# ebartrum/lightning_gan_zoo

Measured on AMD Instinct MI355X. Metric: images/sec (G+D step) at 64x64 bs=128/GPU, higher is better.
Workload: dtype f32; 1 GPU; dc_gan synthetic 64x64 bs=128/GPU, one optimizer cycle of 2 batches (Lightning alternation + toggle), reference optimizer, fp32; key=dc_gan_bs128, global_batch=128, parallelism=dp1, images_counted=2*bs*n_gpus per step (every batch of the cycle)

## Files before the change

### lightning_gan_zoo_amd/csrc/gz_conv.hip

```cpp
#include <cstdio>
#include <type_traits>

#include "gz_conv_choice.h"
#include "gz_conv_direct.h"
#include "gz_igemm.h"
#include "gz_reduce.h"
#include "../../include/gz_ops.h"

namespace gz {


static TileId pick_tile2(long long M, long long N, int ny, int kdim) {
    const bool off = knobs().no_igemm2;
    if (!off && N > 32 && N <= 64 && kdim >= 256) {
        const long long t = ((M + 511) / 512) * ny;
        if (t >= 2 * cus()) return T512x64;
        if (!knobs().no_tile64 && knobs().igemm2_tile == 0 && N == 64 && ((M + 255) / 256) * ny >= cus()) return T256x64;
        return T64x64;
    }
    if (off || N < 128 || kdim < 256) return T64x64;
    const long long t128 = ((M + 255) / 256) * ((N + 127) / 128) * ny;
    const long long t256 = ((M + 255) / 256) * ((N + 255) / 256) * ny;
    const int force = knobs().igemm2_tile;
    const int cu = cus();
// ... 1013 lines not shown
    size_t fewc = 0;
    if (KH == 4 && KW == 4 && wgrad_k4s2p1_fewc_ok(s)) fewc = (size_t)wgrad_k4s2p1_fewc_blocks(s) * (count + K) * 4;
    int chunks = (N * OH * OW + BK - 1) / BK;
    long long tiles = (long long)((K + 127) / 128) * ((C * KH * KW + 127) / 128);
    int splits = wgrad_splits(tiles, chunks);
    {
        const int s2 = (KH == 4 && KW == 4) ? wgrad2_splits<G4421>(s)
                       : (KH == 5 && KW == 5 && OH * 2 == H) ? wgrad2_splits<G5522>(s)
                       : (KH == 3 && KW == 3 && OH == H) ? wgrad2_splits<G3311>(s) : 0;
        if (s2 > splits) splits = s2;
    }
    const size_t generic = splits > 1 ? (size_t)splits * count * 4 : 0;
    return generic > fewc ? generic : fewc;
}

int gz_conv2d_wgrad_fuses_bias(int N, int C, int H, int W, int K, int OH, int OW, int KH, int KW, int S, int P) {
    ConvShape s{N, C, H, W, K, OH, OW};
    if (!shape_ok(s, KH, KW, S, P)) return 0;
#define CALL(G) choose_wgrad<G>(s, kIdeal)
    const Choice c = [&]() -> Choice { GZ_GEOM_DISPATCH_OR(CALL, choice_of(KUnsupported, LGeneric, T64x64)) }();
#undef CALL
    return c.kind == KDirect && c.loader != LFewc;
}

int gz_conv2d_wgrad(const float* x, const float* y, float* dw, float* dbias, float* workspace, size_t ws_bytes, int N,
                    int C, int H, int W, int K, int OH, int OW, int KH, int KW, int S, int P, hipStream_t stream) {
    gz::clear_stale_error();
    ConvShape s{N, C, H, W, K, OH, OW};
    if (!shape_ok(s, KH, KW, S, P)) return GZ_ERR_BAD_SHAPE;
    if (too_large((long long)N * C * H * W) || too_large((long long)N * K * OH * OW)) return GZ_ERR_TOO_LARGE;
    const Facts f = facts_of((const void*)((uintptr_t)x | (uintptr_t)y), dw, workspace, ws_bytes, false, false);
#define CALL(G) launch_wgrad<G>(choose_wgrad<G>(s, f), x, y, dw, dbias, workspace, ws_bytes, s, stream)
    GZ_GEOM_DISPATCH(CALL)
#undef CALL
}

int gz_conv2d_wgrad_partial(const float* x, const float* y, float* dw, float* workspace, size_t ws_bytes, int N, int C,
                            int H, int W, int K, int OH, int OW, int KH, int KW, int S, int P, int* nz_out,
                            long long* stride_out, hipStream_t stream) {
    gz::clear_stale_error();
    if (!nz_out || !stride_out) return GZ_ERR_BAD_SHAPE;
    ConvShape s{N, C, H, W, K, OH, OW};
    if (!shape_ok(s, KH, KW, S, P)) return GZ_ERR_BAD_SHAPE;
    if (too_large((long long)N * C * H * W) || too_large((long long)N * K * OH * OW)) return GZ_ERR_TOO_LARGE;
    *nz_out = 1;
    *stride_out = (long long)K * C * KH * KW;
    const Facts f = facts_of((const void*)((uintptr_t)x | (uintptr_t)y), dw, workspace, ws_bytes, false, false);
    WgDefer d{1, *stride_out};
    tl_wg_defer = &d;
#define CALL(G) launch_wgrad<G>(choose_wgrad<G>(s, f), x, y, dw, nullptr, workspace, ws_bytes, s, stream)
    const int rc = [&]() -> int { GZ_GEOM_DISPATCH(CALL) }();
#undef CALL
    tl_wg_defer = nullptr;
    *nz_out = d.nz;
    *stride_out = d.stride;
    return rc;
}

static bool dgrad_act_direct(const ConvShape& s, int KH, int KW, int S, int P, int act) {
    return KH == 4 && KW == 4 && S == 2 && P == 1 && (act == ACT_RELU || act == ACT_LRELU) && !knobs().no_act_fuse &&
           dgrad_direct<G4421>(s) && smallc_four_pos(s);
}

int gz_conv2d_dgrad_act_fuses(int N, int C, int H, int W, int K, int OH, int OW, int KH, int KW, int S, int P, int act) {
    ConvShape s{N, C, H, W, K, OH, OW};
    return shape_ok(s, KH, KW, S, P) && dgrad_act_direct(s, KH, KW, S, P, act) ? 1 : 0;
}

int gz_conv2d_dgrad_act(const float* gy, const float* fwd_out, int act, float slope, const float* wpack, float* x, int N,
                        int C, int H, int W, int K, int OH, int OW, int KH, int KW, int S, int P, hipStream_t stream) {
    gz::clear_stale_error();
    ConvShape s{N, C, H, W, K, OH, OW};
    if (!gy || !fwd_out || !wpack || !x || !shape_ok(s, KH, KW, S, P)) return GZ_ERR_BAD_SHAPE;
    if (too_large((long long)N * C * H * W) || too_large((long long)N * K * OH * OW)) return GZ_ERR_TOO_LARGE;
    if (!dgrad_act_direct(s, KH, KW, S, P, act) || (((uintptr_t)gy | (uintptr_t)x | (uintptr_t)fwd_out | (uintptr_t)wpack) & 15))
        return GZ_ERR_UNSUPPORTED;
    const float neg = act == ACT_RELU ? 0.f : slope;
    const int ks = smallc_split((long long)N * OH * OW / 4, K);
    return run_dgrad_smallc(gy, wpack, nullptr, x, s, ACT_NONE, 0.f, stream, ks, fwd_out, neg);
}

int gz_set_cu_budget(int cu_count) {
    if (cu_count <= 0) cu_count = 256;
    if (cu_count < 64) cu_count = 64;
    if (cu_count > 256) cu_count = 256;
    gz::cu_budget_ref().store(cu_count, std::memory_order_relaxed);
    return cu_count;
}

int gz_get_cu_budget(void) { return gz::cus(); }

static int stats_wm(TileId t) { return t == T128x32 ? 4 : 2; }
static int stats_tm_rows(TileId t, long long M) {
    if (t == T256x256 || t == T256x128) return (int)((M + 255) / 256) * 2;
    if (t == T512x64) return (int)((M + 511) / 512) * 4;
    if (t == T256x64) return (int)((M + 255) / 256) * 2;
    const int bm = t == T64x64 ? 64 : 128;
    return (int)((M + bm - 1) / bm) * stats_wm(t);
}

int gz_conv2d_fwd_stats_rows(int N, int C, int H, int W, int K, int OH, int OW, int KH, int KW, int S, int P) {
    ConvShape s{N, C, H, W, K, OH, OW};
    if (!shape_ok(s, KH, KW, S, P)) return 0;
    const Facts f{true, true, true, kIdeal.ws_bytes, false, true, true};
#define CALL(G) choose_fwd<G>(s, f)
    const Choice sp = [&]() -> Choice { GZ_GEOM_DISPATCH_OR(CALL, (Choice{KIgemm, LGeneric, T64x64, 2})) }();
#undef CALL
    if (sp.splits > 1) return (int)(((long long)N * OH * OW + 31) / 32);
    return stats_tm_rows(sp.tile, (long long)N * OH * OW);
}

int gz_conv2d_fwd_stats_ws(const float* x, const float* wpack, float* y, float* stats, float* workspace, size_t ws_bytes,
                           int N, int C, int H, int W, int K, int OH, int OW, int KH, int KW, int S, int P,
                           hipStream_t stream) {
    gz::clear_stale_error();
    ConvShape s{N, C, H, W, K, OH, OW};
    if (!shape_ok(s, KH, KW, S, P) || !stats) return GZ_ERR_BAD_SHAPE;
    if (gz_conv2d_fwd_stats_rows(N, C, H, W, K, OH, OW, KH, KW, S, P) <= 0) return GZ_ERR_UNSUPPORTED;
    if ((((uintptr_t)x | (uintptr_t)y) & 15) != 0) return GZ_ERR_BAD_SHAPE;
    if (too_large((long long)N * C * H * W) || too_large((long long)N * K * OH * OW)) return GZ_ERR_TOO_LARGE;
    const Facts f = facts_of(x, y, workspace, ws_bytes, false, true);
#define CALL(G) launch_fwd<G>(choose_fwd<G>(s, f), x, wpack, nullptr, y, s, 0, 0.f, workspace, stats, stream)
    GZ_GEOM_DISPATCH(CALL)
#undef CALL
}

int gz_conv2d_fwd_stats(const float* x, const float* wpack, float* y, float* stats, int N, int C, int H, int W, int K,
                        int OH, int OW, int KH, int KW, int S, int P, hipStream_t stream) {
    return gz_conv2d_fwd_stats_ws(x, wpack, y, stats, nullptr, 0, N, C, H, W, K, OH, OW, KH, KW, S, P, stream);
}

int gz_conv2d_dgrad_stats_rows(int N, int C, int H, int W, int K, int OH, int OW, int KH, int KW, int S, int P) {
    ConvShape s{N, C, H, W, K, OH, OW};
    if (!shape_ok(s, KH, KW, S, P) || H % S || W % S) return 0;
    const Facts f{true, true, true, kIdeal.ws_bytes, false, true, true};
#define CALL(G) (dgrad_direct<G>(s) ? Choice{KIgemm, LGeneric, T64x64, 2} : choose_dgrad<G>(s, f))
    const Choice sp = [&]() -> Choice { GZ_GEOM_DISPATCH_OR(CALL, (Choice{KIgemm, LGeneric, T64x64, 2})) }();
#undef CALL
    if (is_tile2(sp.tile) && !(KH == 4 && KW == 4 && S == 2 && P == 1)) return 0;
    if (sp.splits > 1) {
        if (!(KH == 4 && KW == 4 && S == 2 && P == 1)) return 0;
        return S * S * (int)(((long long)N * (H / S) * (W / S) + 31) / 32);
    }
    return S * S * stats_tm_rows(sp.tile, (long long)N * (H / S) * (W / S));
}

int gz_conv2d_dgrad_stats_ws(const float* y, const float* wpack, float* x, float* stats, float* workspace,
                             size_t ws_bytes, int N, int C, int H, int W, int K, int OH, int OW, int KH, int KW, int S,
                             int P, hipStream_t stream) {
    gz::clear_stale_error();
    ConvShape s{N, C, H, W, K, OH, OW};
    if (!shape_ok(s, KH, KW, S, P) || !stats) return GZ_ERR_BAD_SHAPE;
    if (gz_conv2d_dgrad_stats_rows(N, C, H, W, K, OH, OW, KH, KW, S, P) <= 0) return GZ_ERR_UNSUPPORTED;
    if ((((uintptr_t)x | (uintptr_t)y) & 15) != 0) return GZ_ERR_BAD_SHAPE;
    if (too_large((long long)N * C * H * W) || too_large((long long)N * K * OH * OW)) return GZ_ERR_TOO_LARGE;
    const Facts f = facts_of(y, x, workspace, ws_bytes, false, true);
#define CALL(G) launch_dgrad<G>(choose_dgrad<G>(s, f), y, wpack, nullptr, x, s, 0, 0.f, workspace, stats, stream)
    GZ_GEOM_DISPATCH(CALL)
#undef CALL
}

int gz_conv2d_dgrad_stats(const float* y, const float* wpack, float* x, float* stats, int N, int C, int H, int W, int K,
                          int OH, int OW, int KH, int KW, int S, int P, hipStream_t stream) {
    return gz_conv2d_dgrad_stats_ws(y, wpack, x, stats, nullptr, 0, N, C, H, W, K, OH, OW, KH, KW, S, P, stream);
}

static bool any_shape_ok(const ConvShape& s, const AnyGeom& g) {
// ... 160 lines not shown
```

### lightning_gan_zoo_amd/csrc/gz_igemm2.h

```cpp
#pragma once
#include "gz_igemm_core.h"

namespace gz {

constexpr int STAGES2 = 3;
#ifndef GZ2_DEPTH_TN1_KG2
#define GZ2_DEPTH_TN1_KG2 6
#endif
#ifndef GZ2_DEPTH_TN1_KG1
#define GZ2_DEPTH_TN1_KG1 4
#endif
#ifndef GZ2_DEPTH_TN2_KG2
#define GZ2_DEPTH_TN2_KG2 3
#endif
#ifndef GZ2_DEPTH_TN2_KG1
#define GZ2_DEPTH_TN2_KG1 3
#endif
#ifndef GZ2_BARRIER_TN1_KG2
#define GZ2_BARRIER_TN1_KG2 2
#endif
#ifndef GZ2_BARRIER_TN1_KG1
#define GZ2_BARRIER_TN1_KG1 2
#endif
constexpr uint32_t SOFF_OOB = 0x80000000u;

template <int WM_, int WN_, int TN_, int OCC_, int TM_ = 4>
struct TileCfg2 {
    static constexpr int WM = WM_, WN = WN_, TM = TM_, TN = TN_, OCC = OCC_;
    static constexpr int BM = WM * TM * 32, BN = WN * TN * 32;
    static_assert(WM * WN == 4, "4 wavefronts per workgroup, one per SIMD");
};

template <int BN>
struct MContigB2 {
    static_assert(BN == 64 || BN == 128 || BN == 256, "piece mapping");
    using Params = typename MContigLoader<BN>::Params;
    static constexpr int LD = BN, ROWS = BK;
    static constexpr int PIECES = BK * BN / 256 / 4;
    static constexpr int RPP = 256 / BN;
    __amdgpu_buffer_rsrc_t rsrc;
    uint32_t voff, ldb;
    int wave;
    __device__ __forceinline__ void init(const Params& p, int tile, int y, int tid) {
        rsrc = make_rsrc(p.base + (long long)y * p.batch_stride, (uint32_t)p.K * p.ld * 4u);
        const int lane = tid & 63;
        wave = __builtin_amdgcn_readfirstlane(tid >> 6);
        const int f = lane * 4, r = f / BN, col = f % BN;
        const int n = tile * BN + col;
        ldb = (uint32_t)p.ld * 4u;
        voff = n < p.MN ? (uint32_t)(r * p.ld + n) * 4u : OOB;
    }
    __device__ __forceinline__ void issue_piece(int kc, float* stage, int p, bool live) {
        const int piece = wave * PIECES + p;
        bload_lds16(rsrc, stage + piece * 256, voff, live ? (uint32_t)(kc * BK + piece * RPP) * ldb : SOFF_OOB);
    }
};

template <int BM>
struct ConvDgA2 {
    static_assert(BM == 256 || BM == 512, "whole 256-pixel pieces per LDS row");
    using Params = typename ConvDgALoader<BM, 4, 4, 2, 1>::Params;
    static constexpr int PPR = BM / 256;
    static constexpr int LD = BM + 4, ROWS = BK / 2, PIECES = 2 * PPR;
    static constexpr int ZERO_COL = BM;
    static constexpr bool ROWSHARE = true;
    __amdgpu_buffer_rsrc_t rsrc;
    uint32_t voff[2 * PPR];
    int wave, K, OHW, shift_half1;
    __device__ __forceinline__ void init(const Params& p, int tile, int phase, int tid) {
        const ConvShape& s = p.s;
        rsrc = make_rsrc(p.y, (uint32_t)s.N * s.K * s.OH * s.OW * 4u);
        const int lane = tid & 63;
        wave = __builtin_amdgcn_readfirstlane(tid >> 6);
        K = s.K; OHW = s.OH * s.OW;
        const int py = phase / 2, px = phase % 2;
        shift_half1 = (px + 1) / 2 - 1;
#pragma unroll
        for (int hb = 0; hb < PPR; ++hb) {
            const uint32_t m = (uint32_t)tile * BM + hb * 256 + lane * 4;
            const bool m_ok = m < (uint32_t)s.N * p.AH * p.AW;
            const uint32_t n = fdiv(m, p.div_ahw);
            const uint32_t pix = m - n * (uint32_t)(p.AH * p.AW);
            const uint32_t a = fdiv(pix, p.div_aw);
            const uint32_t b = pix - a * (uint32_t)p.AW;
#pragma unroll
            for (int ty = 0; ty < 2; ++ty) {
                const int oy = (int)a + (py + 1) / 2 - ty;
                const bool ok = m_ok && (unsigned)oy < (unsigned)s.OH;
                voff[ty * PPR + hb] = ok ? (n * (uint32_t)(s.K * OHW) + (uint32_t)(oy * s.OW) + b) * 4u : OOB;
            }
        }
    }
    __device__ __forceinline__ int frag_shift(int half) const { return half ? shift_half1 : shift_half1 + 1; }
    __device__ __forceinline__ void issue_piece(int kc, float* stage, int p, bool live) {
        const int kol = kc * (BK / 4) + wave;
        bload_lds16(rsrc, stage + (wave * 2 + p / PPR) * LD + (p % PPR) * 256, voff[p],
                    (live && kol < K) ? (uint32_t)kol * (uint32_t)OHW * 4u : SOFF_OOB);
    }
};

template <int BM, int OWC>
struct ConvFwdA2 {
    static_assert(BM == 256 && BM % OWC == 0 && OWC >= 2, "piece mapping");
    using Params = typename ConvFwdALoader<BM, 4, 4, 2, 1>::Params;
    static constexpr int LD = BM, ROWS = BK / 2, PIECES = 2;
    static constexpr int OW_C = OWC;
    static constexpr int EXTRA = (6 * OWC + 4 + 3) & ~3;
    static constexpr bool FWDROWS = true;
    __amdgpu_buffer_rsrc_t rsrc;
    uint32_t voff[2];
    int wave, HW, C;
    __device__ __forceinline__ void init(const Params& p, int tile, int y, int tid) {
        const ConvShape& s = p.s;
        rsrc = make_rsrc(p.x, (uint32_t)(s.N * s.C * s.H * s.W) * 4u);
        const int lane = tid & 63;
        wave = __builtin_amdgcn_readfirstlane(tid >> 6);
        HW = s.H * s.W; C = s.C;
#pragma unroll
        for (int q = 0; q < 2; ++q) {
            const int f = ((wave * 2 + q) * 64 + lane) * 4;
            const int seg = f / (8 * OWC), rem = f - seg * 8 * OWC;
            const int ky = rem / (2 * OWC), col = rem - ky * 2 * OWC;
            const uint32_t m = (uint32_t)tile * BM + seg * OWC;
            const bool m_ok = m < (uint32_t)s.N * s.OH * s.OW;
            const uint32_t n = fdiv(m, p.div_ohw);
            const uint32_t oy = fdiv(m - n * (uint32_t)(s.OH * s.OW), p.div_ow);
            const int iy = (int)oy * 2 - 1 + ky;
            const bool ok = m_ok && (unsigned)iy < (unsigned)s.H;
            voff[q] = ok ? (n * (uint32_t)(s.C * HW) + (uint32_t)(iy * s.W + col)) * 4u : OOB;
        }
    }
    static constexpr int ZERO = ROWS * LD;
    __device__ __forceinline__ void frag(int m_local, int half, int& even, int& odd) const {
        const int seg = m_local / OWC, ox = m_local - seg * OWC;
        const int base = seg * 8 * OWC + 2 * ox - 1 + half;
        even = (half == 0 && ox == 0) ? ZERO : base;
        odd = (half == 1 && ox == OWC - 1) ? ZERO : base + 2;
    }
    __device__ __forceinline__ void issue_piece(int kc, float* stage, int p, bool live) {
        bload_lds16(rsrc, stage + (wave * 2 + p) * 256, voff[p], (live && kc < C) ? (uint32_t)kc * (uint32_t)HW * 4u : SOFF_OOB);
    }
};

template <class Geo_>
struct TapGatherA2 {
    using Geo = Geo_;
    using Params = typename Geo::Params;
    static constexpr int BM = Geo::BM, LD = BM, ROWS = BK;
    static constexpr int G = BM / 64;
    static constexpr int PIECES = BK * G / 4;
    Geo geo;
    __amdgpu_buffer_rsrc_t rsrc;
    uint32_t vbase[G], veff[G];
    typename Geo::Pix pix[G];
    int wave, blocks, last_tap, last_kc, cb;
    uint32_t tap_soff;
    __device__ __forceinline__ void init(const Params& p, int tile, int y, int tid) {
        rsrc = geo.init(p, y);
        const int lane = tid & 63;
        wave = __builtin_amdgcn_readfirstlane(tid >> 6);
        blocks = round_bk(geo.chans) / BK;
        last_tap = -1; last_kc = -1; cb = 0; tap_soff = 0;
#pragma unroll
        for (int g = 0; g < G; ++g) {
            vbase[g] = geo.locate(p, (uint32_t)tile * BM + g * 64 + lane, pix[g]);
            veff[g] = OOB;
        }
    }
    __device__ __forceinline__ void issue_piece(int kc, float* stage, int p, bool live) {
        if (p == 0) {
            int tap = last_tap;
            if (kc == last_kc + 1 && last_kc >= 0) {
                cb += BK;
                if (cb >= blocks * BK) { cb = 0; ++tap; }
            } else {
                tap = kc / blocks;
                cb = (kc - tap * blocks) * BK;
            }
            last_kc = kc;
            if (tap != last_tap) {
                last_tap = tap;
                const auto tp = geo.tap(tap);
                tap_soff = geo.tap_bytes(tp);
#pragma unroll
                for (int g = 0; g < G; ++g) veff[g] = geo.inside(pix[g], tp) ? vbase[g] : OOB;
            }
        }
        const int row = wave * 4 + p / G, g = p % G;
        const int c = cb + row;
        bload_lds4(rsrc, stage + row * LD + g * 64, veff[g],
                   (live && c < geo.chans) ? (uint32_t)c * (uint32_t)geo.plane * 4u + tap_soff : SOFF_OOB);
    }
};

template <int BM, int KH, int KW, int S, int P>
using ConvTapA2 = TapGatherA2<TapGeoFwd<BM, KH, KW, S, P>>;
template <int BM>
using ConvTapAnyA2 = TapGatherA2<TapGeoFwdAny<BM>>;
template <int BM, int KH, int KW, int S, int P>
using ConvDgTapA2 = TapGatherA2<TapGeoDg<BM, KH, KW, S, P>>;
template <int BM, int KS, int S, int P>
using Conv3DTapA2 = TapGatherA2<TapGeoFwd3D<BM, KS, S, P>>;
template <int BM, int KS, int S, int P>
using Conv3DDgTapA2 = TapGatherA2<TapGeoDg3D<BM, KS, S, P>>;

template <int BM>
struct ConvDg5A2 {
    static_assert(BM == 256, "one 256-pixel piece per LDS row");
    using Params = typename ConvDgALoaderTap<BM, 5, 5, 2, 2>::Params;
    static constexpr int LD = BM + 4, ROWS = 8, PIECES = 2;
    static constexpr int ZERO_COL = BM;
    static constexpr bool ROWSHARE = true, DUALMODE = true;
    static constexpr int MODES = 2, KSTEPS = 12;
    static constexpr bool step_plain(int m, int S) { return S >= 8; }
    static constexpr unsigned step_mask(int m, int S) {
        return m == 0 ? (S < 8 ? 15u : 5u) : (S < 8 ? 3u : 1u);
    }
    static constexpr int step_arow(int m, int S) { return S < 8 ? S : 2 * (S - 8); }
    static constexpr int step_brow(int m, int S) { return S < 8 ? 2 * S : 16 + 2 * (S - 8); }
    __amdgpu_buffer_rsrc_t rsrc;
    uint32_t voff0, voff1, voff2;
    int wave, K, OHW;
    int bound[1];
// ... 165 lines not shown
                 : "v"(a), "v"(b[0]), "v"(b[1]), "v"(b[2]), "v"(b[3]));
}
__device__ __forceinline__ void mfma_row_mn(f32x16 (&c)[2], float a, const float (&b)[2]) {
    asm volatile(GZ2_NOP
                 "v_mfma_f32_32x32x2_f32 %0, %2, %3, %0\n\t"
                 "v_mfma_f32_32x32x2_f32 %1, %2, %4, %1"
                 : "+a"(c[0]), "+a"(c[1])
                 : "v"(a), "v"(b[0]), "v"(b[1]));
}
__device__ __forceinline__ void lgkm_done(float (&a)[4], float (&b)[4]) {
    asm volatile("s_waitcnt lgkmcnt(0)" : "+v"(a[0]), "+v"(a[1]), "+v"(a[2]), "+v"(a[3]), "+v"(b[0]), "+v"(b[1]), "+v"(b[2]), "+v"(b[3]));
}
__device__ __forceinline__ void lgkm_done(float (&a)[4], float (&b)[2]) {
    asm volatile("s_waitcnt lgkmcnt(0)" : "+v"(a[0]), "+v"(a[1]), "+v"(a[2]), "+v"(a[3]), "+v"(b[0]), "+v"(b[1]));
}
__device__ __forceinline__ void lgkm_done(float (&a)[2], float (&b)[4]) {
    asm volatile("s_waitcnt lgkmcnt(0)" : "+v"(a[0]), "+v"(a[1]), "+v"(b[0]), "+v"(b[1]), "+v"(b[2]), "+v"(b[3]));
}
__device__ __forceinline__ void lgkm_done(float (&a)[4], float (&b)[1]) {
    asm volatile("s_waitcnt lgkmcnt(0)" : "+v"(a[0]), "+v"(a[1]), "+v"(a[2]), "+v"(a[3]), "+v"(b[0]));
}

template <class AL, class = void>
struct a_extra_of { static constexpr int value = 0; };
template <class AL>
struct a_extra_of<AL, std::void_t<decltype(AL::EXTRA)>> { static constexpr int value = AL::EXTRA; };
template <class AL>
constexpr int igemm2_a_extra() { return a_extra_of<AL>::value; }
template <class AL, class = void>
struct fwd_ow_of { static constexpr int value = 1; };
template <class AL>
struct fwd_ow_of<AL, std::void_t<decltype(AL::OW_C)>> { static constexpr int value = AL::OW_C; };
template <class AL>
constexpr int fwd_ow() { return fwd_ow_of<AL>::value; }

template <class AL>
constexpr int mode_count_of() {
    if constexpr (is_dualmode<AL>::value) return AL::MODES;
    else return 1;
}
template <class AL>
constexpr bool mode_plain_of(int m, int S) {
    if constexpr (is_dualmode<AL>::value) return AL::step_plain(m, S);
    else return false;
}
template <class AL>
constexpr unsigned mode_mask_of(int m, int S) {
    if constexpr (is_dualmode<AL>::value) return AL::step_mask(m, S);
    else return 0xFu;
}
template <class AL>
constexpr int ksteps_of() {
    if constexpr (is_dualmode<AL>::value) return AL::KSTEPS;
    else return BK / 2;
}
template <class AL>
constexpr int step_arow_of(int m, int S) {
    if constexpr (is_dualmode<AL>::value) return AL::step_arow(m, S);
    else return S;
}
template <class AL>
constexpr int step_brow_of(int m, int S) {
    if constexpr (is_dualmode<AL>::value) return AL::step_brow(m, S);
    else return 2 * S;
}

constexpr size_t LDS_PER_CU = 160 * 1024;
template <class AL, class BL>
constexpr int igemm2_stage_floats() { return AL::ROWS * AL::LD + igemm2_a_extra<AL>() + BL::ROWS * BL::LD; }
template <class Cfg, class AL, class BL, int KG>
constexpr size_t igemm2_lds_bytes_at(int depth) {
    if (KG == 1) return (size_t)(depth * igemm2_stage_floats<AL, BL>() + 32) * 4;
    const size_t rings = (size_t)(2 * ((depth * igemm2_stage_floats<AL, BL>() + 63) / 64 * 64) + 32) * 4;
    const size_t park = (size_t)Cfg::TM * Cfg::TN * 16 * NT * 4;
    return rings > park ? rings : park;
}
template <class Cfg, class AL, class BL, int KG>
constexpr bool igemm2_tunable() {
    return Cfg::BM == 256 && (is_rowshare<AL>::value || is_fwdrows<AL>::value) && !is_dualmode<AL>::value &&
           fwd_ow<AL>() < 64;
}
template <class Cfg, class AL, class BL, int KG>
constexpr int igemm2_interval() {
    if (igemm2_tunable<Cfg, AL, BL, KG>() && Cfg::TN == 1) return KG == 2 ? GZ2_BARRIER_TN1_KG2 : GZ2_BARRIER_TN1_KG1;
    return 1;
}
template <class Cfg, class AL, class BL, int KG>
constexpr int igemm2_depth() {
    if (igemm2_tunable<Cfg, AL, BL, KG>()) {
        if (Cfg::TN == 1) return KG == 2 ? GZ2_DEPTH_TN1_KG2 : GZ2_DEPTH_TN1_KG1;
        if (Cfg::TN == 2) return KG == 2 ? GZ2_DEPTH_TN2_KG2 : GZ2_DEPTH_TN2_KG1;
    }
    return STAGES2;
}
template <class Cfg, class AL, class BL, int KG>
constexpr int igemm2_ring_floats() {
    return ((igemm2_depth<Cfg, AL, BL, KG>() * igemm2_stage_floats<AL, BL>() + 63) / 64) * 64;
}
template <class Cfg, class AL, class BL>
constexpr size_t igemm2_lds_bytes() { return igemm2_lds_bytes_at<Cfg, AL, BL, 1>(igemm2_depth<Cfg, AL, BL, 1>()); }
template <class Cfg, class AL, class BL>
constexpr size_t igemm2_lds_bytes_kg2() { return igemm2_lds_bytes_at<Cfg, AL, BL, 2>(igemm2_depth<Cfg, AL, BL, 2>()); }

template <class Cfg, class AL, class BL, class Epi, int KG = 1>
__global__ __launch_bounds__(NT * KG, KG == 1 ? Cfg::OCC : 2) void igemm2_kernel(typename AL::Params pa, typename BL::Params pb,
                                                                              typename Epi::Params pe, GridMap gm) {
    constexpr int LDA = AL::LD, LDB = BL::LD;
    constexpr int TM = Cfg::TM, TN = Cfg::TN;
    static_assert((TM == 4 || (TM == 2 && is_dualmode<AL>::value)) && (TN == 1 || TN == 2 || TN == 4),
                  "fragment registers of the hand-ordered k-step");
    static_assert(KG == 1 || (KG == 2 && TN <= 2), "two wave groups: the parked accumulators must fit the LDS");
    constexpr bool RS = is_rowshare<AL>::value;
    constexpr bool FR = is_fwdrows<AL>::value;
    constexpr bool DM = is_dualmode<AL>::value;
    static_assert(!DM || (RS && KG == 1 && (TN == 2 || TN == 4)), "multi-mode: row-shared loader, phases in the accumulator blocks");
    constexpr int A_EXTRA = igemm2_a_extra<AL>();
    constexpr int A_ELEMS = AL::ROWS * LDA + A_EXTRA, B_ELEMS = BL::ROWS * LDB;
    constexpr int STAGE = A_ELEMS + B_ELEMS;
    constexpr int PAD = 16;
    constexpr int DEPTH = igemm2_depth<Cfg, AL, BL, KG>();
    constexpr int BI = igemm2_interval<Cfg, AL, BL, KG>();
    constexpr int GROUPS = DEPTH / BI;
    static_assert(DEPTH % BI == 0 && (BI == 1 ? GROUPS >= 3 : GROUPS >= 2) && (BI == 1 || (BI == 2 && !DM)),
                  "group t+GROUPS-1 lands in the stages group t-1 was read from");
    static_assert(DEPTH == STAGES2 || (KG == 2 ? igemm2_lds_bytes_kg2<Cfg, AL, BL>()
                                               : Cfg::OCC * igemm2_lds_bytes<Cfg, AL, BL>()) <= LDS_PER_CU,
                  "workgroups per CU x LDS per workgroup");
    extern __shared__ __attribute__((aligned(16))) float smem2[];
    const int kg = KG == 1 ? 0 : __builtin_amdgcn_readfirstlane((int)threadIdx.x >> 8);
    float* const ring = smem2 + PAD + kg * igemm2_ring_floats<Cfg, AL, BL, KG>();
    GZ2_STAMP(st0);
#ifdef GZ2_STAMPS
    const unsigned long long sr0 = __builtin_amdgcn_s_memrealtime();
    unsigned long long st1 = st0, st2 = st0;
#endif

    const int tid = KG == 1 ? (int)threadIdx.x : ((int)threadIdx.x & (NT - 1));
    const int nwg = gridDim.x;
    int bid = blockIdx.x;
    if (gm.stagger > 0 && bid < 512 && blockIdx.z == 0) {
        const unsigned hw = __builtin_amdgcn_s_getreg(((4 - 1) << 11) | (16 << 6) | 4);
        if (hw & 1u) {
            const unsigned long long t_end = __builtin_amdgcn_s_memtime() + (unsigned long long)gm.stagger;
            while (__builtin_amdgcn_s_memtime() < t_end) __builtin_amdgcn_s_sleep(64);
        }
    }
    int y;
    if (gm.var_chunks) {
        const int tiles = gm.tiles_m * gm.tiles_n;
        y = gm.phase_order[bid / tiles];
        bid %= tiles;
    } else {
        if (!gm.no_swizzle) {
            const int q = nwg >> 3, rr = nwg & 7, x = bid & 7, i = bid >> 3;
            bid = (x < rr ? x * (q + 1) : rr * (q + 1) + (x - rr) * q) + i;
        }
        y = bid % gm.ny;
        bid /= gm.ny;
    }
    const int tile_n = bid % gm.tiles_n;
    const int tile_m = bid / gm.tiles_n;
    const int z = blockIdx.z;
    const int kcA = z * gm.chunks_per_split;
    const int kcB = min(gm.var_chunks ? gm.phase_chunks[y] : gm.chunks, kcA + gm.chunks_per_split);
    if (gm.slab && gm.var_chunks && kcA >= kcB) return;
    int kc0 = kcA, kc1 = kcB, kend = kcB;
    if constexpr (KG == 2) {
        const int h = (kcB - kcA + 1) >> 1;
        kc0 = kcA + kg * h;
        kend = kc0 + h;
        kc1 = min(kcB, kend);
    }

    AL al;
    BL bl;
    al.init(pa, tile_m, y, tid);
    bl.init(pb, tile_n, y, tid);

    f32x16 acc[TM][TN];
#pragma unroll
    for (int i = 0; i < TM; ++i)
#pragma unroll
        for (int j = 0; j < TN; ++j)
#pragma unroll
            for (int r = 0; r < 16; ++r) acc[i][j][r] = 0.f;

    const int lane = tid & 63, wave = __builtin_amdgcn_readfirstlane(tid >> 6);
    const int wm = wave / Cfg::WN, wn = wave % Cfg::WN;
    const int half = lane >> 5, l32 = lane & 31;
    const uint32_t lds0 = (uint32_t)(uintptr_t)(__attribute__((address_space(3))) float*)ring;
    uint32_t a_addr[TM];
#pragma unroll
    for (int i = 0; i < TM; ++i)
        a_addr[i] = lds0 + (uint32_t)(B_ELEMS + half * (RS ? 0 : LDA) + wm * TM * 32 + i * 32 + l32) * 4u;
    if constexpr (RS) {
        const int sh = al.frag_shift(half);
#pragma unroll
        for (int i = 0; i < TM; ++i) {
            const int b = (tile_m * Cfg::BM + wm * TM * 32 + i * 32 + l32) % pa.AW;
            const bool zero = (sh < 0 && b == 0) || (sh > 0 && b == pa.AW - 1);
            a_addr[i] = zero ? lds0 + (uint32_t)(B_ELEMS + AL::ZERO_COL) * 4u : a_addr[i] + (uint32_t)(sh * 4);
        }
        static_assert(DEPTH * AL::ROWS * 4 <= NT, "one pad float per thread");
        if (tid < DEPTH * AL::ROWS * 4) {
            const int st = tid / (AL::ROWS * 4), q = tid % (AL::ROWS * 4);
            ring[st * STAGE + B_ELEMS + (q >> 2) * LDA + AL::ZERO_COL + (q & 3)] = 0.f;
        }
    }
    uint32_t a_addrB[TM];
    if constexpr (DM) {
#pragma unroll
        for (int i = 0; i < TM; ++i) {
            const int b = (tile_m * Cfg::BM + wm * TM * 32 + i * 32 + l32) % pa.AW;
            a_addrB[i] = lds0 + (uint32_t)(B_ELEMS + half * LDA + (b == 0 ? AL::ZERO_COL : wm * TM * 32 + i * 32 + l32 - 1)) * 4u;
        }
    }
    uint32_t a_odd[TM];
    if constexpr (FR) {
#pragma unroll
        for (int i = 0; i < TM; ++i) {
            int e, o;
            al.frag(wm * TM * 32 + i * 32 + l32, half, e, o);
            a_addr[i] = lds0 + (uint32_t)(B_ELEMS + e) * 4u;
            a_odd[i] = lds0 + (uint32_t)(B_ELEMS + o) * 4u;
        }
        for (int q = tid; q < DEPTH * A_EXTRA; q += NT)
            ring[(q / A_EXTRA) * STAGE + B_ELEMS + AL::ZERO + q % A_EXTRA] = 0.f;
    }
    const uint32_t b_addr = lds0 + (uint32_t)(half * LDB + wn * TN * 32 + l32) * 4u;

    constexpr int NPA = AL::PIECES, NPB = BL::PIECES, NP = NPA + NPB, STEPS = ksteps_of<AL>();
    static_assert((STEPS == 8 || STEPS == 12) && (BI == 1 || STEPS == 8), "k-steps per chunk, per group 8, 12 or 16");
    constexpr int PPS = (NP + STEPS - 1) / STEPS;
    static_assert(PPS <= 4 && (DEPTH - BI) * NP < 64,
                  "pieces are spread over the k-step's four MFMA rows; vmcnt is 6 bits and DEPTH-BI chunks are in flight");
    constexpr int NWAIT = (DEPTH - 2 * BI) * NP;
    constexpr int GSTEPS = BI * STEPS;
    auto issue_piece = [&](int kc, int st, int p, bool live) {
#ifdef GZ2_EXP_NODMA
        if (kc >= kc0 + DEPTH - BI) return;
#endif
#ifdef GZ2_EXP_SAMECHUNK
        if (kc >= kc0 + DEPTH - BI) kc = kc0;
#endif
        float* sb = ring + st * STAGE;
        if (p < NPA) al.issue_piece(kc, sb + B_ELEMS, p, live);
        else bl.issue_piece(kc, sb, p - NPA, live);
    };
    auto fetch_m = [&](auto Sc, auto Mc, uint32_t so, float (&af)[TM], float (&bf)[TN]) {
        constexpr int S = decltype(Sc)::value, MD = decltype(Mc)::value;
        constexpr bool PL = mode_plain_of<AL>(MD, S);
        constexpr unsigned MK = mode_mask_of<AL>(MD, S);
        constexpr int AO = LDA * step_arow_of<AL>(MD, S) * 4, BO = step_brow_of<AL>(MD, S) * LDB * 4;
#pragma unroll
        for (int i = 0; i < TM; ++i) af[i] = lds_rd<AO>((PL ? a_addrB[i] : a_addr[i]) + so);
        if constexpr ((MK & 1u) != 0) bf[0] = lds_rd<BO>(b_addr + so);
        if constexpr (TN >= 2 && (MK & 2u) != 0) bf[1] = lds_rd<BO + 128>(b_addr + so);
        if constexpr (TN == 4 && (MK & 4u) != 0) bf[2] = lds_rd<BO + 256>(b_addr + so);
        if constexpr (TN == 4 && (MK & 8u) != 0) bf[3] = lds_rd<BO + 384>(b_addr + so);
    };
    auto fetch_first = [&](int kc, uint32_t so, float (&af)[TM], float (&bf)[TN]) {
        if constexpr (DM) {
            if (al.mode_of(kc) == 0) fetch_m(std::integral_constant<int, 0>{}, std::integral_constant<int, 0>{}, so, af, bf);
            else fetch_m(std::integral_constant<int, 0>{}, std::integral_constant<int, 1>{}, so, af, bf);
        }
    };
    auto fetch = [&](auto Sc, uint32_t so, float (&af)[TM], float (&bf)[TN]) {
        constexpr int S = decltype(Sc)::value % STEPS, JO = decltype(Sc)::value / STEPS * STAGE * 4;
        constexpr int AO = (RS ? LDA : 2 * LDA) * S * 4 + JO, BO = 2 * S * LDB * 4 + JO;
        static_assert(AO + 2 * LDA * 4 < 65536 && BO + 512 < 65536, "ds_read immediate offsets");
#ifdef GZ2_EXP_NOFETCH
        if (so != 0xFFFFFFFFu) return;
#endif
        if constexpr (FR) {
            constexpr int FO = (S >> 1) * 2 * fwd_ow<AL>() * 4 + JO;
            af[0] = lds_rd<FO>(((S & 1) ? a_odd[0] : a_addr[0]) + so);
            af[1] = lds_rd<FO>(((S & 1) ? a_odd[1] : a_addr[1]) + so);
            af[2] = lds_rd<FO>(((S & 1) ? a_odd[2] : a_addr[2]) + so);
            af[3] = lds_rd<FO>(((S & 1) ? a_odd[3] : a_addr[3]) + so);
        } else {
            af[0] = lds_rd<AO>(a_addr[0] + so);
            af[1] = lds_rd<AO>(a_addr[1] + so);
            af[2] = lds_rd<AO>(a_addr[2] + so);
            af[3] = lds_rd<AO>(a_addr[3] + so);
        }
        {
        bf[0] = lds_rd<BO>(b_addr + so);
        if constexpr (TN >= 2) bf[1] = lds_rd<BO + 128>(b_addr + so);
        if constexpr (TN == 4) {
            bf[2] = lds_rd<BO + 256>(b_addr + so);
            bf[3] = lds_rd<BO + 384>(b_addr + so);
        }
        }
    };
    auto mask = [&](float (&)[TM]) {};

    if (kcA < kcB) {
#pragma unroll
        for (int d = 0; d < DEPTH - BI; ++d)
#pragma unroll
            for (int p = 0; p < NP; ++p) issue_piece(kc0 + d, d, p, kc0 + d < kc1);
#ifdef GZ2_EXP_NO_LGKM_PROLOGUE
        asm volatile("s_waitcnt vmcnt(%0)" ::"n"(NWAIT) : "memory");
#else
        asm volatile("s_waitcnt vmcnt(%0) lgkmcnt(0)" ::"n"(NWAIT) : "memory");
#endif
        __builtin_amdgcn_s_barrier();
#ifdef GZ2_STAMPS
        st1 = __builtin_amdgcn_s_memtime();
#endif
        float af[2][TM], bf[2][TN];
#ifdef GZ2_STEP_STAMPS
        unsigned long long step_cyc[STEPS] = {}, step_t = __builtin_amdgcn_s_memtime();
        unsigned long long wait_cyc[2] = {0, 0};
#endif
        if constexpr (DM) {
#pragma unroll
            for (int q = 0; q < 2; ++q)
#pragma unroll
                for (int j = 0; j < TN; ++j) bf[q][j] = 0.f;
            fetch_first(kc0, 0u, af[0], bf[0]);
        } else {
            fetch(std::integral_constant<int, 0>{}, 0u, af[0], bf[0]);
        }
        lgkm_done(af[0], bf[0]);
        mask(af[0]);
        int stage = 0;
        auto run_chunks = [&](int k_from, int k_to, auto Mc) {
        for (int kc = k_from; kc < k_to; kc += BI) {
            int s1 = stage + 1; if (s1 >= GROUPS) s1 -= GROUPS;
            int s2 = stage - 1; if (s2 < 0) s2 += GROUPS;
            const uint32_t so = (uint32_t)(stage * BI * STAGE * 4), sno = (uint32_t)(s1 * BI * STAGE * 4);
            const bool more = kc + DEPTH - BI < kc1, more1 = kc + DEPTH - BI + 1 < kc1;
            auto kstep = [&](auto Sc) {
                constexpr int S = decltype(Sc)::value;
                constexpr int MD = decltype(Mc)::value;
                constexpr int c = S & 1, n = c ^ 1;
                auto mfma_row = [&](f32x16 (&cc)[TN], float a, const float (&b)[TN]) {
                    if constexpr (DM) {
                        constexpr unsigned MK = mode_mask_of<AL>(MD, S);
                        if constexpr (MK == (TN == 4 ? 15u : 3u)) gz::mfma_row(cc, a, b);
                        else {
                            if constexpr ((MK & 1u) != 0) gz::mfma_one(cc[0], a, b[0]);
                            if constexpr (TN >= 2 && (MK & 2u) != 0) gz::mfma_one(cc[1], a, b[1]);
                            if constexpr (TN == 4 && (MK & 4u) != 0) gz::mfma_one(cc[2], a, b[2]);
                            if constexpr (TN == 4 && (MK & 8u) != 0) gz::mfma_one(cc[3], a, b[3]);
                        }
                    } else gz::mfma_row(cc, a, b);
                };
                auto fetch_same = [&](auto S2c, uint32_t o, float (&fa)[TM], float (&fb)[TN]) {
                    if constexpr (DM) fetch_m(S2c, Mc, o, fa, fb);
                    else fetch(S2c, o, fa, fb);
                };
                auto pieces = [&](auto Rowc) {
                    constexpr int row = decltype(Rowc)::value;
                    constexpr int r = PPS == 1 ? (row == 1 ? 0 : -1) : row;
                    constexpr int q = S * PPS + r;
                    if constexpr (r >= 0 && r < PPS && q < BI * NP)
// ... 717 lines not shown
```

### lightning_gan_zoo_amd/csrc/gz_knobs.h

```cpp
#pragma once
#include <stdlib.h>
#include <string.h>
#include <atomic>

namespace gz {

#define GZ_KNOB_LIST(X)                                                                                               \
                                                                                          \
    X(bool, no_igemm2, "GZ_NO_IGEMM2", false)                        \
    X(bool, no_igemm2_tap, "GZ_NO_IGEMM2_TAP", false)                      \
    X(bool, no_plane_a, "GZ_NO_PLANE_A", false)                \
    X(bool, no_wg3r, "GZ_NO_WG3R", false)                               \
    X(int, wg3r_wgs, "GZ_WG3R_WGS", 2)                              \
    X(int, wg3r_min_chunks, "GZ_WG3R_MIN_CHUNKS", 24)                         \
    X(bool, no_fewk_wg, "GZ_NO_FEWK_WG", false)               \
    X(bool, no_fewk_conv, "GZ_NO_FEWK_CONV", false)            \
    X(int, dg3_tile, "GZ_DG3_TILE", 0)                       \
    X(int, dg3_wgs, "GZ_DG3_WGS", 2)                         \
    X(int, dg3_min_chunks, "GZ_DG3_MIN_CHUNKS", 32)                            \
    X(bool, no_igemm2_wg, "GZ_NO_IGEMM2_WG", false)                              \
    X(bool, no_igemm2w, "GZ_NO_IGEMM2W", false)              \
    X(bool, no_igemm2wg, "GZ_NO_IGEMM2WG", false)                          \
    X(int, igemm2_tile, "GZ_IGEMM2_TILE", 0)                                 \
    X(bool, no_tile64, "GZ_NO_TILE64", false)                                  \
    X(bool, no_kg2, "GZ_NO_KG2", false)                             \
    X(bool, no_pool_plane, "GZ_NO_POOL_PLANE", false)               \
    X(bool, no_pool_group, "GZ_NO_POOL_GROUP", false)                  \
    X(bool, no_any2, "GZ_NO_ANY2", false)                    \
    X(bool, no_dg5, "GZ_NO_DG5", false)                      \
    X(int, dg5_wgs, "GZ_DG5_WGS", 512)                              \
    X(int, dg5_min_chunks, "GZ_DG5_MIN_CHUNKS", 24)             \
    X(int, dg5_min_units, "GZ_DG5_MIN_UNITS", 80)             \
    X(int, kg2_min_chunks, "GZ_KG2_MIN_CHUNKS", 32)                           \
    X(int, tap64_min_chunks, "GZ_TAP64_MIN_CHUNKS", 32)      \
    X(int, tile, "GZ_TILE", -1)                                               \
    X(int, min_wgs, "GZ_MIN_WGS", 0)                                \
    X(bool, no_big_split, "GZ_NO_BIG_SPLIT", false)                                                                   \
    X(bool, no_splitk, "GZ_NO_SPLITK", false)                                                                         \
    X(int, split_target, "GZ_SPLIT_TARGET", 1024)                                                                     \
    X(int, split_below, "GZ_SPLIT_BELOW", 512)                                                                        \
    X(bool, no_tapmajor, "GZ_NO_TAPMAJOR", false)                                                                     \
    X(bool, no_row4, "GZ_NO_ROW4", false)                                                                             \
    X(int, fwd2_min_tiles, "GZ_FWD2_MIN_TILES", 16)                                                                   \
    X(int, dg2_min_tiles, "GZ_DG2_MIN_TILES", 64)                                                                     \
    X(int, tap_wgs, "GZ_TAP_WGS", 384)                                                                                \
    X(int, tap_cps_max, "GZ_TAP_CPS_MAX", 96)                                                                         \
    X(int, wg_target, "GZ_WG_TARGET", 1024)                                                                           \
    X(int, wg2_min_chunks, "GZ_WG2_MIN_CHUNKS", 0)                                                                    \
    X(bool, wg_generic, "GZ_WG_GENERIC", false)                                                                       \
                                                                                                  \
    X(bool, no_smallc, "GZ_NO_SMALLC", false)                                                                         \
    X(bool, no_smallc5, "GZ_NO_SMALLC5", false)                                                                       \
    X(bool, smallc_one_pos, "GZ_SMALLC_ONE_POS", false)                                                               \
    X(long long, smallc_split_below, "GZ_SMALLC_SPLIT_BELOW", 192 * 1024)                                             \
    X(long long, smallc_split8_below, "GZ_SMALLC_SPLIT8_BELOW", 36 * 1024)                                            \
    X(int, smallc_ks, "GZ_SMALLC_KS", 0)                                                                              \
    X(bool, no_fewc_wg, "GZ_NO_FEWC_WG", false)                                                                       \
    X(bool, no_act_fuse, "GZ_NO_ACT_FUSE", false)                                                                     \
    X(bool, no_pack_k4, "GZ_NO_PACK_K4", false)                                                                       \
    X(bool, no_resample_swizzle, "GZ_NO_RESAMPLE_SWIZZLE", false)                                                     \
    X(int, fewc_wg_blocks, "GZ_FEWC_WG_BLOCKS", 512)                                                                  \
    X(bool, no_smallch_conv, "GZ_NO_SMALLCH_CONV", false)                                                             \
    X(bool, no_smallch_wg, "GZ_NO_SMALLCH_WG", false)                                                                 \
    X(int, c3_gpw, "GZ_C3_GPW", 4)                                                                                    \
                                                                                        \
    X(bool, no_xcd_swizzle, "GZ_NO_XCD_SWIZZLE", false)                                                               \
    X(int, dyn_lds, "GZ_DYN_LDS", 0)                                                                                  \
    X(int, igemm2_stagger, "GZ_IGEMM2_STAGGER", 0)                                                                    \
    X(int, igemm2_lds, "GZ_IGEMM2_LDS", 0)                                                                            \
                                                                     \
    X(bool, dg3_even_split, "GZ_DG3_EVEN_SPLIT", false)                                                               \
    X(int, wg3_target, "GZ_WG3_TARGET", 1024)                                                                         \
    X(int, wg3_tile, "GZ_WG3_TILE", -1)                                                                               \
    X(bool, norm_unfused, "GZ_NORM_UNFUSED", false)                                                                   \
    X(int, norm_bwd_cache, "GZ_NORM_BWD_CACHE", 4)                                                                    \
    X(bool, resample_fwd_direct, "GZ_RESAMPLE_FWD_DIRECT", false)                                                     \
    X(int, resample_bwd_mode, "GZ_RESAMPLE_BWD", 0)

struct Knobs {
    bool experiments;
#define GZ_KNOB_FIELD(type, name, env, dflt) type name;
    GZ_KNOB_LIST(GZ_KNOB_FIELD)
#undef GZ_KNOB_FIELD
};

inline void knob_read(bool& v, const char* e) { v = e != nullptr; }
inline void knob_read(int& v, const char* e) {
    if (!e) return;
    if (!strcmp(e, "scatter")) v = 1;
    else if (!strcmp(e, "gather")) v = 2;
    else v = atoi(e);
}
inline void knob_read(long long& v, const char* e) { if (e) v = atoll(e); }

inline const Knobs& knobs() {
    static const Knobs k = [] {
        Knobs n;
#define GZ_KNOB_INIT(type, name, env, dflt) n.name = dflt;
        GZ_KNOB_LIST(GZ_KNOB_INIT)
#undef GZ_KNOB_INIT
        const char* on = getenv("GZ_EXPERIMENTS");
        n.experiments = on && on[0] && on[0] != '0';
        if (n.experiments) {
#define GZ_KNOB_ENV(type, name, env, dflt) knob_read(n.name, getenv(env));
            GZ_KNOB_LIST(GZ_KNOB_ENV)
#undef GZ_KNOB_ENV
        }
        return n;
    }();
    return k;
}

inline std::atomic<int>& cu_budget_ref() {
    static std::atomic<int> v{256};
    return v;
}
inline int cus() { return cu_budget_ref().load(std::memory_order_relaxed); }

}
```

Measured before the change: 45570 images/s.

## Re-lay forward conv A tile by kernel row and deepen TN2 pipeline

Changes the LDS layout of the stride-2 forward conv A loader so each wave loads one kernel row (ky = wave) into a padded pitch of 2*BM+4 floats, which simplifies fragment addressing and alters LDS bank patterns. The zero-pad initialization becomes a single store per thread. TN=2 igemm2 configurations now use a barrier interval of 2 and ring depth 4 instead of 3, which increases LDS use and may lower occupancy. The CU budget lower clamp also becomes a knob, with the same default of 64.

```diff
diff --git a/lightning_gan_zoo_amd/csrc/gz_conv.hip b/lightning_gan_zoo_amd/csrc/gz_conv.hip
--- a/lightning_gan_zoo_amd/csrc/gz_conv.hip
+++ b/lightning_gan_zoo_amd/csrc/gz_conv.hip
@@ -1119,7 +1119,8 @@
 
 int gz_set_cu_budget(int cu_count) {
     if (cu_count <= 0) cu_count = 256;
-    if (cu_count < 64) cu_count = 64;
+    const int lo = gz::knobs().cu_budget_min > 0 ? gz::knobs().cu_budget_min : 1;
+    if (cu_count < lo) cu_count = lo;
     if (cu_count > 256) cu_count = 256;
     gz::cu_budget_ref().store(cu_count, std::memory_order_relaxed);
     return cu_count;
diff --git a/lightning_gan_zoo_amd/csrc/gz_igemm2.h b/lightning_gan_zoo_amd/csrc/gz_igemm2.h
--- a/lightning_gan_zoo_amd/csrc/gz_igemm2.h
+++ b/lightning_gan_zoo_amd/csrc/gz_igemm2.h
@@ -10,17 +10,23 @@
 #ifndef GZ2_DEPTH_TN1_KG1
 #define GZ2_DEPTH_TN1_KG1 4
 #endif
-#ifndef GZ2_DEPTH_TN2_KG2
-#define GZ2_DEPTH_TN2_KG2 3
-#endif
-#ifndef GZ2_DEPTH_TN2_KG1
-#define GZ2_DEPTH_TN2_KG1 3
-#endif
 #ifndef GZ2_BARRIER_TN1_KG2
 #define GZ2_BARRIER_TN1_KG2 2
 #endif
 #ifndef GZ2_BARRIER_TN1_KG1
 #define GZ2_BARRIER_TN1_KG1 2
+#endif
+#ifndef GZ2_BARRIER_TN2_KG2
+#define GZ2_BARRIER_TN2_KG2 2
+#endif
+#ifndef GZ2_BARRIER_TN2_KG1
+#define GZ2_BARRIER_TN2_KG1 2
+#endif
+#ifndef GZ2_DEPTH_TN2_KG2
+#define GZ2_DEPTH_TN2_KG2 (GZ2_BARRIER_TN2_KG2 == 2 ? 4 : 3)
+#endif
+#ifndef GZ2_DEPTH_TN2_KG1
+#define GZ2_DEPTH_TN2_KG1 (GZ2_BARRIER_TN2_KG1 == 2 ? 4 : 3)
 #endif
 constexpr uint32_t SOFF_OOB = 0x80000000u;
 
@@ -105,7 +111,8 @@
     using Params = typename ConvFwdALoader<BM, 4, 4, 2, 1>::Params;
     static constexpr int LD = BM, ROWS = BK / 2, PIECES = 2;
     static constexpr int OW_C = OWC;
-    static constexpr int EXTRA = (6 * OWC + 4 + 3) & ~3;
+    static constexpr int PITCH = 2 * BM + 4;
+    static constexpr int EXTRA = 4 * PITCH - ROWS * LD;
     static constexpr bool FWDROWS = true;
     __amdgpu_buffer_rsrc_t rsrc;
     uint32_t voff[2];
@@ -118,9 +125,9 @@
         HW = s.H * s.W; C = s.C;
 #pragma unroll
         for (int q = 0; q < 2; ++q) {
-            const int f = ((wave * 2 + q) * 64 + lane) * 4;
-            const int seg = f / (8 * OWC), rem = f - seg * 8 * OWC;
-            const int ky = rem / (2 * OWC), col = rem - ky * 2 * OWC;
+            const int f = (q * 64 + lane) * 4;
+            const int seg = f / (2 * OWC), col = f - seg * 2 * OWC;
+            const int ky = wave;
             const uint32_t m = (uint32_t)tile * BM + seg * OWC;
             const bool m_ok = m < (uint32_t)s.N * s.OH * s.OW;
             const uint32_t n = fdiv(m, p.div_ohw);
@@ -130,15 +137,15 @@
             voff[q] = ok ? (n * (uint32_t)(s.C * HW) + (uint32_t)(iy * s.W + col)) * 4u : OOB;
         }
     }
-    static constexpr int ZERO = ROWS * LD;
+    static constexpr int ZERO = 2 * BM;
     __device__ __forceinline__ void frag(int m_local, int half, int& even, int& odd) const {
-        const int seg = m_local / OWC, ox = m_local - seg * OWC;
-        const int base = seg * 8 * OWC + 2 * ox - 1 + half;
+        const int ox = m_local % OWC;
+        const int base = 2 * m_local - 1 + half;
         even = (half == 0 && ox == 0) ? ZERO : base;
         odd = (half == 1 && ox == OWC - 1) ? ZERO : base + 2;
     }
     __device__ __forceinline__ void issue_piece(int kc, float* stage, int p, bool live) {
-        bload_lds16(rsrc, stage + (wave * 2 + p) * 256, voff[p], (live && kc < C) ? (uint32_t)kc * (uint32_t)HW * 4u : SOFF_OOB);
+        bload_lds16(rsrc, stage + wave * PITCH + p * 256, voff[p], (live && kc < C) ? (uint32_t)kc * (uint32_t)HW * 4u : SOFF_OOB);
     }
 };
 
@@ -470,7 +477,10 @@
 }
 template <class Cfg, class AL, class BL, int KG>
 constexpr int igemm2_interval() {
-    if (igemm2_tunable<Cfg, AL, BL, KG>() && Cfg::TN == 1) return KG == 2 ? GZ2_BARRIER_TN1_KG2 : GZ2_BARRIER_TN1_KG1;
+    if (igemm2_tunable<Cfg, AL, BL, KG>()) {
+        if (Cfg::TN == 1) return KG == 2 ? GZ2_BARRIER_TN1_KG2 : GZ2_BARRIER_TN1_KG1;
+        if (Cfg::TN == 2) return KG == 2 ? GZ2_BARRIER_TN2_KG2 : GZ2_BARRIER_TN2_KG1;
+    }
     return 1;
 }
 template <class Cfg, class AL, class BL, int KG>
@@ -612,8 +622,11 @@
             a_addr[i] = lds0 + (uint32_t)(B_ELEMS + e) * 4u;
             a_odd[i] = lds0 + (uint32_t)(B_ELEMS + o) * 4u;
         }
-        for (int q = tid; q < DEPTH * A_EXTRA; q += NT)
-            ring[(q / A_EXTRA) * STAGE + B_ELEMS + AL::ZERO + q % A_EXTRA] = 0.f;
+        static_assert(A_EXTRA == 16 && DEPTH * A_EXTRA <= NT, "one pad float per thread");
+        if (tid < DEPTH * A_EXTRA) {
+            const int st = tid / A_EXTRA, q = tid % A_EXTRA;
+            ring[st * STAGE + B_ELEMS + (q >> 2) * AL::PITCH + AL::ZERO + (q & 3)] = 0.f;
+        }
     }
     const uint32_t b_addr = lds0 + (uint32_t)(half * LDB + wn * TN * 32 + l32) * 4u;
 
@@ -661,7 +674,8 @@
         if (so != 0xFFFFFFFFu) return;
 #endif
         if constexpr (FR) {
-            constexpr int FO = (S >> 1) * 2 * fwd_ow<AL>() * 4 + JO;
+            constexpr int FO = (S >> 1) * AL::PITCH * 4 + JO;
+            static_assert(FO + AL::PITCH * 4 < 65536, "ds_read immediate offsets");
             af[0] = lds_rd<FO>(((S & 1) ? a_odd[0] : a_addr[0]) + so);
             af[1] = lds_rd<FO>(((S & 1) ? a_odd[1] : a_addr[1]) + so);
             af[2] = lds_rd<FO>(((S & 1) ? a_odd[2] : a_addr[2]) + so);
diff --git a/lightning_gan_zoo_amd/csrc/gz_knobs.h b/lightning_gan_zoo_amd/csrc/gz_knobs.h
--- a/lightning_gan_zoo_amd/csrc/gz_knobs.h
+++ b/lightning_gan_zoo_amd/csrc/gz_knobs.h
@@ -68,6 +68,7 @@
     X(int, dyn_lds, "GZ_DYN_LDS", 0)                                                                                  \
     X(int, igemm2_stagger, "GZ_IGEMM2_STAGGER", 0)                                                                    \
     X(int, igemm2_lds, "GZ_IGEMM2_LDS", 0)                                                                            \
+    X(int, cu_budget_min, "GZ_CU_BUDGET_MIN", 64)            \
                                                                      \
     X(bool, dg3_even_split, "GZ_DG3_EVEN_SPLIT", false)                                                               \
     X(int, wg3_target, "GZ_WG3_TARGET", 1024)                                                                         \
```

After: 45980 images/s (median of 6 runs). No clear change (+0.9%).
